# serycjon/MFT

Measured on AMD Instinct MI355X. Metric: tracked frames/sec at 512x512, 12 RAFT iters; flow EPE vs reference, higher is better.
Workload: dtype f32 (update-block products as split fp16 x 3 on the fp16 matrix cores, fp32 accumulation; error per product <= ~2^-23, see DESIGN.md section 4 and parity below); 1 GPU; MFT.track on synthetic 512x512 video, deltas [inf,1,2,4,8,16,32], 7/7.00/7 (min/mean/max) flow pairs per timed frame, 12 RAFT iters, seeded synthetic weights (BASELINE.json configs[1]); parallelism=single GPU, frames_resident_in_hbm=True, preroll_frames=32

## Files before the change

mft_amd/csrc/volume_tile.hip:

```cpp
#include "common.h"
#include "profile.h"
#include "device_prims.h"

namespace mftx {

constexpr int VT_C = 256;
constexpr int VT_ROW = VT_C * 4 + 16;
constexpr int VT_TARGETS = 128 * VT_ROW;
constexpr int VT_LDS = VT_TARGETS + 8 * 1024;

struct VolTileArgs {
    const float *f1;
    const float *f2s;
    float *lvl0, *lvl1, *lvl2, *lvl3;
    long long s0, s1, s2, s3;
    int P, N, h, w, sbw, n_sb, wb0;
    float scale;
    int qchunks, blocks_per_chunk;
    int ablate;
    int gathered;
    long long f2_bstride;
    PairPtrs f1p;
};

template <int N>
__device__ __forceinline__ float vt_shl(float v) {
    return __builtin_bit_cast(float, __builtin_amdgcn_update_dpp(0, __builtin_bit_cast(int, v), 0x100 + N, 0xf, 0xf, true));
}
template <int N>
__device__ __forceinline__ float vt_shr(float v) {
    return __builtin_bit_cast(float, __builtin_amdgcn_update_dpp(0, __builtin_bit_cast(int, v), 0x110 + N, 0xf, 0xf, true));
}

template <bool QSPLIT>
__global__ __launch_bounds__(512, 2) void volume_tile_kernel(VolTileArgs p) {
    extern __shared__ __attribute__((aligned(16))) unsigned char vt_lds[];
    unsigned char *lds = vt_lds;
    const int tid = (int)threadIdx.x, lane = tid & 63, wv = __builtin_amdgcn_readfirstlane(tid >> 6);
    const int wg = (int)blockIdx.x;
    const int qc = wg % p.qchunks, sb = (wg / p.qchunks) % p.n_sb, bz = wg / (p.qchunks * p.n_sb);
    const int sby = sb / p.sbw, sbx = sb - sby * p.sbw;
    const float k2048 = __builtin_bit_cast(float, __builtin_amdgcn_readfirstlane(0x45000000));

    {
        const float *f2p = p.f2s + (long long)bz * p.f2_bstride;
#pragma unroll 4
        for (int k = 0; k < 16; ++k) {
            const int q = k * 512 + tid, m = q >> 6, pc = q & 63;
            const int j = m >> 5, mm = m & 31;
            const int ty = 8 * sby + 4 * (j >> 1) + (mm >> 3), tx = 16 * sbx + 8 * (j & 1) + (mm & 7);
            uint4 v = make_uint4(0u, 0u, 0u, 0u);
            if (ty < p.h && tx < p.w) v = *reinterpret_cast<const uint4 *>(f2p + ((long long)ty * p.w + tx) * VT_C + pc * 4);
            *reinterpret_cast<uint4 *>(lds + m * VT_ROW + pc * 16) = v;
        }
    }
    lds_barrier();

    const unsigned char *abase = lds + (lane & 31) * VT_ROW + (lane >> 5) * 32;
    const int n_blocks = (p.N + 31) >> 5;
    const int b_lo = qc * p.blocks_per_chunk, b_hi = (b_lo + p.blocks_per_chunk < n_blocks) ? b_lo + p.blocks_per_chunk : n_blocks;
    const long long qbase = (long long)bz * p.N;
    const float inv2048 = 1.f / 2048.f;
    const int hf = lane >> 5;
    const int h2 = p.h >> 2, w2 = p.w >> 2, h3 = p.h >> 3, w3 = p.w >> 3;

    const int pp = lane & 31;
    const int l1_src = 4 * (32 * hf + 2 * (pp & 3) + 16 * ((pp >> 3) & 1) + ((pp >> 2) & 1) + 8 * (pp >> 4));
    const int l3_src = 4 * ((lane + 16) & 63);
    constexpr int PF = 3;
    f32x4 raw[PF][2];
    const float *f1base = p.gathered ? p.f1p.p[bz] : p.f1 + qbase * VT_C;
    auto row_of = [&](int qb) {
        const int q = qb * 32 + (lane & 31);
        return f1base + (long long)(q < p.N ? q : p.N - 1) * VT_C + 8 * hf;
    };
    auto prefetch = [&](const float *src) {
#pragma unroll
        for (int g = 0; g < PF; ++g) {
            raw[g][0] = *reinterpret_cast<const f32x4 *>(src + 16 * g);
            raw[g][1] = *reinterpret_cast<const f32x4 *>(src + 16 * g + 4);
        }
    };
    if (b_lo + wv < b_hi) prefetch(row_of(b_lo + wv));
    for (int qb = b_lo + wv; qb < b_hi; qb += 8) {
        const float *src = row_of(qb);
        f32x16 acc[4], accx[4];
#pragma unroll
        for (int j = 0; j < 4; ++j)
#pragma unroll
            for (int r = 0; r < 16; ++r) { acc[j][r] = 0.f; accx[j][r] = 0.f; }
        f16x8 ah[2][4], al[2][4];
        auto read_a = [&](int g, int set) {
#pragma unroll
            for (int j = 0; j < 4; ++j) {
                ah[set][j] = *reinterpret_cast<const f16x8 *>(abase + j * 32 * VT_ROW + g * 64);
                al[set][j] = *reinterpret_cast<const f16x8 *>(abase + j * 32 * VT_ROW + g * 64 + 16);
            }
        };
        read_a(0, 0);
#pragma unroll
        for (int g = 0; g < 16; ++g) {
            const int set = g & 1;
            f16x8 bh, bl;
            if constexpr (QSPLIT) {
                bh = __builtin_bit_cast(f16x8, raw[g % PF][0]);
                bl = __builtin_bit_cast(f16x8, raw[g % PF][1]);
            } else split8(raw[g % PF][0], raw[g % PF][1], k2048, bh, bl);
            __builtin_amdgcn_sched_barrier(0);
            if (g + 1 < 16) read_a(g + 1, set ^ 1);
            if (g + PF < 16) {
                raw[g % PF][0] = *reinterpret_cast<const f32x4 *>(src + 16 * (g + PF));
                raw[g % PF][1] = *reinterpret_cast<const f32x4 *>(src + 16 * (g + PF) + 4);
            }
            __builtin_amdgcn_sched_barrier(0);
#pragma unroll
            for (int j = 0; j < 4; ++j) acc[j] = mfma_f16(bh, ah[set][j], acc[j]);
#pragma unroll
            for (int j = 0; j < 4; ++j) accx[j] = mfma_f16(bh, al[set][j], accx[j]);
#pragma unroll
            for (int j = 0; j < 4; ++j) accx[j] = mfma_f16(bl, ah[set][j], accx[j]);
            __builtin_amdgcn_sched_barrier(0);
        }

        if (qb + 8 < b_hi) prefetch(row_of(qb + 8));
        __builtin_amdgcn_sched_barrier(0);

        const int m = lane & 31;
        const int q0 = qb * 32;
        const long long blk0 = ((long long)(2 * sby) * p.wb0 + 2 * sbx) * 32 + m;
        const int rows_ok = p.N - q0 < 32 ? p.N - q0 : 32;
        const __amdgpu_buffer_rsrc_t r0 = __builtin_amdgcn_make_buffer_rsrc(p.lvl0 + (qbase + q0) * p.s0, 0, (unsigned)((long long)rows_ok * p.s0 * 4), 0x00020000);
        const __amdgpu_buffer_rsrc_t r1 = __builtin_amdgcn_make_buffer_rsrc(p.lvl1 + (qbase + q0) * p.s1, 0, (unsigned)((long long)rows_ok * p.s1 * 4), 0x00020000);
        const unsigned v1off = (unsigned)((4 * hf * p.s1 + ((long long)sby * p.sbw + sbx) * 32 + m) * 4);
        const unsigned s0b = (unsigned)(p.s0 * 4), s1b = (unsigned)(p.s1 * 4), jrow = (unsigned)(p.wb0 * 128);
        int le = lane;
        asm volatile("" : "+v"(le));
        const int d2c = le & 7, d2hf = (le >> 3) & 1, d2i = le >> 4;
        const int l2_pull = 4 * (32 * d2hf + 16 * (d2c >> 2) + 2 * (d2c & 3));
        const int l2_y = 2 * sby + (d2c >> 2), l2_x = 4 * sbx + (d2c & 3);
        const bool l2_ok = l2_y < h2 && l2_x < w2;
        const int l2_off = l2_y * w2 + l2_x, l2_row = 4 * d2hf + d2i;
        const int d3c = le & 1, d3hf = (le >> 1) & 1, d3r = le >> 2;
        const int l3_pull = 4 * (32 * d3hf + 4 * d3c);
        const int l3_x = 2 * sbx + d3c;
        const bool l3_ok = sby < h3 && l3_x < w3;
        const int l3_off = sby * w3 + l3_x, l3_row = 8 * (d3r >> 2) + 4 * d3hf + (d3r & 3);
        float *slab = reinterpret_cast<float *>(lds + VT_TARGETS + wv * 1024);
        const unsigned v0off4 = (unsigned)((le >> 3) * s0b) + (unsigned)((blk0 - m) * 4) + (unsigned)(le & 7) * 16u;
        float acc2 = 0.f, acc3 = 0.f;
#pragma unroll
        for (int g = 0; g < 4; ++g) {
#ifdef MFTX_TUNING
            const bool st0g = !(p.ablate & 1);
#else
            const bool st0g = true;
#endif
            float vv[4][4];
#pragma unroll
            for (int i = 0; i < 4; ++i)
#pragma unroll
                for (int j = 0; j < 4; ++j) vv[i][j] = (acc[j][4 * g + i] + accx[j][4 * g + i] * inv2048) * p.scale;
            f32x4 line[4];
#pragma unroll
            for (int j = 0; j < 4; ++j) {
#pragma unroll
                for (int i = 0; i < 4; ++i) slab[(4 * hf + i) * 32 + m] = vv[i][j];
                line[j] = *reinterpret_cast<const f32x4 *>(slab + (le >> 3) * 32 + (le & 7) * 4);
            }
            if (st0g) {
#pragma unroll
                for (int j = 0; j < 4; ++j)
                    __builtin_amdgcn_raw_buffer_store_b128(__builtin_bit_cast(u32x4, line[j]), r0, v0off4 + (j >> 1) * jrow + (j & 1) * 128u, (unsigned)(8 * g) * s0b, 0);
            }
#pragma unroll
        for (int i = 0; i < 4; ++i) {
            const int r = 4 * g + i;
            const int qrow = q0 + 8 * (r >> 2) + 4 * hf + (r & 3);
            const bool row_ok = qrow < p.N;
#ifdef MFTX_TUNING
            const bool st1 = row_ok && !(p.ablate & 2);
#define MFTX_VT_ST23 (!(p.ablate & 10))
#else
            const bool st1 = row_ok;
#define MFTX_VT_ST23 true
#endif
            float merged = 0.f;
#pragma unroll
            for (int j = 0; j < 4; ++j) {
                const float v = vv[i][j];
                float t = v + vt_shl<1>(v);
                t = t + vt_shl<8>(v);
                t = (t + vt_shl<9>(v)) * 0.25f;
                if (j == 0) merged = t;
                else {
                    float sh = j == 1 ? vt_shr<1>(t) : (j == 2 ? vt_shr<8>(t) : vt_shr<9>(t));
                    asm volatile("" : "+v"(sh));
                    const bool take = j == 1 ? (m & 1) != 0 : (j == 2 ? ((m >> 3) & 1) && !(m & 1) : ((m >> 3) & 1) && (m & 1));
                    merged = take ? sh : merged;
                }
            }
            const float l1 = __builtin_bit_cast(float, __builtin_amdgcn_ds_bpermute(l1_src, __builtin_bit_cast(int, merged)));
            if (st1) __builtin_amdgcn_raw_buffer_store_b32(__builtin_bit_cast(unsigned, l1), r1, v1off, (unsigned)(8 * (r >> 2) + (r & 3)) * s1b, 0);
            float t2 = l1 + vt_shl<1>(l1);
            t2 = t2 + vt_shl<8>(l1);
            t2 = (t2 + vt_shl<9>(l1)) * 0.25f;
            asm volatile("" : "+v"(t2));
            {
                const float pulled = __builtin_bit_cast(float, __builtin_amdgcn_ds_bpermute(l2_pull, __builtin_bit_cast(int, t2)));
                acc2 = d2i == (r & 3) ? pulled : acc2;
                if ((r & 3) == 3) {
                    const int row2 = q0 + 8 * (r >> 2) + l2_row;
                    if (MFTX_VT_ST23 && l2_ok && row2 < p.N) p.lvl2[(qbase + row2) * p.s2 + l2_off] = acc2;
                }
            }
            const float bq = vt_shl<2>(t2);
            const float cq = __builtin_bit_cast(float, __builtin_amdgcn_ds_bpermute(l3_src, __builtin_bit_cast(int, t2)));
            const float dq = __builtin_bit_cast(float, __builtin_amdgcn_ds_bpermute(l3_src + 8, __builtin_bit_cast(int, t2)));
            float v3 = (((t2 + bq) + cq) + dq) * 0.25f;
            asm volatile("" : "+v"(v3));
            {
                const float pulled = __builtin_bit_cast(float, __builtin_amdgcn_ds_bpermute(l3_pull, __builtin_bit_cast(int, v3)));
                acc3 = d3r == r ? pulled : acc3;
                if (r == 15) {
                    const int row3 = q0 + l3_row;
                    if (MFTX_VT_ST23 && l3_ok && row3 < p.N) p.lvl3[(qbase + row3) * p.s3 + l3_off] = acc3;
                }
            }
        }
        }
    }
}

static int vt_num_cus() {
    static const int n = [] {
        int dev = 0, cus = 256;
        hipDeviceProp_t prop;
        if (hipGetDevice(&dev) == hipSuccess && hipGetDeviceProperties(&prop, dev) == hipSuccess && prop.multiProcessorCount > 0) cus = prop.multiProcessorCount;
        return cus;
    }();
    return n;
}

bool volume_tile_applicable(int C) { return C == VT_C; }

__global__ void vt_query_split_kernel(const float *__restrict__ in, uint4 *__restrict__ out, long long n8) {
    const long long i = (long long)blockIdx.x * blockDim.x + threadIdx.x;
    const float k2048 = __builtin_bit_cast(float, __builtin_amdgcn_readfirstlane(0x45000000));
    if (i >= n8) return;
    const f32x4 u = *reinterpret_cast<const f32x4 *>(in + i * 8), v = *reinterpret_cast<const f32x4 *>(in + i * 8 + 4);
    f16x8 hi, lo;
    split8(u, v, k2048, hi, lo);
    out[2 * i] = __builtin_bit_cast(uint4, hi);
    out[2 * i + 1] = __builtin_bit_cast(uint4, lo);
}

int launch_volume_query_split(const float *in, void *out, long long n, hipStream_t s) {
    if (n <= 0 || n % 8) return fail(MFTX_E_ARG, "volume_query_split: a positive multiple of 8 floats");
    if (!aligned16(in) || !aligned16(out)) return fail(MFTX_E_ALIGN, "volume_query_split: operands must be 16-byte aligned");
    const long long n8 = n / 8;
    hipLaunchKernelGGL(vt_query_split_kernel, dim3((unsigned)((n8 + 255) / 256)), dim3(256), 0, s, in, reinterpret_cast<uint4 *>(out), n8);
    return check_launch("volume_query_split");
}

int launch_volume_tile(const float *f1, const float *f2s, int P, int h, int w, float *const lvl[4], hipStream_t s, const PairPtrs *f1p, long long f2_bstride,
                       bool f1_split) {
    if (f1p && P > MFTX_MAX_GATHER) return fail(MFTX_E_ARG, "corr_pyramid: at most %d gathered pairs", MFTX_MAX_GATHER);
    const PyramidLayout L = pyramid_layout(h, w);
    VolTileArgs a{};
    a.f1 = f1; a.f2s = f2s; a.lvl0 = lvl[0]; a.lvl1 = lvl[1]; a.lvl2 = lvl[2]; a.lvl3 = lvl[3];
    a.s0 = L.stride[0]; a.s1 = L.stride[1]; a.s2 = L.stride[2]; a.s3 = L.stride[3];
    a.P = P; a.N = h * w; a.h = h; a.w = w; a.sbw = L.sbw; a.n_sb = L.sbh * L.sbw; a.wb0 = L.wb[0];
    a.scale = 1.0f / sqrtf((float)VT_C);
    a.gathered = f1p ? 1 : 0;
    if (f1p) a.f1p = *f1p;
    a.f2_bstride = f2_bstride >= 0 ? f2_bstride : (long long)a.N * VT_C;
    const int n_blocks = (a.N + 31) / 32;
    const long long base = (long long)P * a.n_sb;
    a.ablate = tune_env("MFTX_VT_ABLATE", 0);
    static const int q_forced = tune_env("MFTX_VT_QCHUNKS", 0);
    int qchunks = q_forced > 0 ? q_forced : (base * 4 >= 3LL * vt_num_cus() ? 1 : (int)((vt_num_cus() + base - 1) / base));
    if (qchunks < 1) qchunks = 1;
    if (qchunks > (n_blocks + 7) / 8) qchunks = (n_blocks + 7) / 8;
    a.blocks_per_chunk = (n_blocks + qchunks - 1) / qchunks;
    a.qchunks = (n_blocks + a.blocks_per_chunk - 1) / a.blocks_per_chunk;
    const long long wgs = base * a.qchunks;
    if (wgs > 0x7fffffffLL) return fail(MFTX_E_ARG, "corr_pyramid: too many workgroups");
    static bool attr_set = false;
    if (!attr_set) {
        if (hipFuncSetAttribute(reinterpret_cast<const void *>(volume_tile_kernel<false>), hipFuncAttributeMaxDynamicSharedMemorySize, VT_LDS) != hipSuccess ||
            hipFuncSetAttribute(reinterpret_cast<const void *>(volume_tile_kernel<true>), hipFuncAttributeMaxDynamicSharedMemorySize, VT_LDS) != hipSuccess)
            return fail(MFTX_E_STATE, "corr_pyramid: cannot reserve %d bytes of LDS", VT_LDS);
        attr_set = true;
    }
    ProfScope prof(PC_CORR_VOLUME, s, 2.0 * a.N * a.N * (double)VT_C * P);
    if (f1_split) hipLaunchKernelGGL(volume_tile_kernel<true>, dim3((unsigned)wgs), dim3(512), VT_LDS, s, a);
    else hipLaunchKernelGGL(volume_tile_kernel<false>, dim3((unsigned)wgs), dim3(512), VT_LDS, s, a);
    return check_launch("volume_tile");
}

}
```

Measured before the change: 187.4 frames/s.

## Deepen query prefetch ring, reorder MFMA/LDS reads, vectorize level-1 stores

Enlarges the per-wave prefetch ring of query feature loads from 3 to 8 k-groups. The ring now rolls over into the next query block instead of reloading it at the end of the loop. A-operand LDS reads drop from double buffering to single buffers for the high and low halves, interleaved between the MFMA groups, which reduces register pressure. Level-1 pyramid outputs are staged through an LDS slab and written as 128-bit buffer stores instead of scalar stores, and the lvl0/lvl1 stores now carry a cache policy flag (value 2). The aim is to hide global load latency, widen the stores and cut write cache pollution, at the cost of more VGPRs for the ring and a changed row-bounds check that relies on the buffer resource limit.

```diff
diff --git a/mft_amd/csrc/volume_tile.hip b/mft_amd/csrc/volume_tile.hip
--- a/mft_amd/csrc/volume_tile.hip
+++ b/mft_amd/csrc/volume_tile.hip
@@ -8,6 +8,7 @@
 constexpr int VT_ROW = VT_C * 4 + 16;
 constexpr int VT_TARGETS = 128 * VT_ROW;
 constexpr int VT_LDS = VT_TARGETS + 8 * 1024;
+constexpr int VT_STORE_POLICY = 2;
 
 struct VolTileArgs {
     const float *f1;
@@ -61,80 +62,77 @@
     const int b_lo = qc * p.blocks_per_chunk, b_hi = (b_lo + p.blocks_per_chunk < n_blocks) ? b_lo + p.blocks_per_chunk : n_blocks;
     const long long qbase = (long long)bz * p.N;
     const float inv2048 = 1.f / 2048.f;
-    const int hf = lane >> 5;
     const int h2 = p.h >> 2, w2 = p.w >> 2, h3 = p.h >> 3, w3 = p.w >> 3;
 
-    const int pp = lane & 31;
-    const int l1_src = 4 * (32 * hf + 2 * (pp & 3) + 16 * ((pp >> 3) & 1) + ((pp >> 2) & 1) + 8 * (pp >> 4));
-    const int l3_src = 4 * ((lane + 16) & 63);
-    constexpr int PF = 3;
+    constexpr int PF = 8;
+    static_assert(16 % PF == 0, "the ring must close over a query block's 16 k groups");
     f32x4 raw[PF][2];
-    const float *f1base = p.gathered ? p.f1p.p[bz] : p.f1 + qbase * VT_C;
+    const unsigned char *f1base = reinterpret_cast<const unsigned char *>(p.gathered ? p.f1p.p[bz] : p.f1 + qbase * VT_C);
+    auto lane_again = [] { return (int)__builtin_amdgcn_mbcnt_hi(~0u, __builtin_amdgcn_mbcnt_lo(~0u, 0u)); };
     auto row_of = [&](int qb) {
-        const int q = qb * 32 + (lane & 31);
-        return f1base + (long long)(q < p.N ? q : p.N - 1) * VT_C + 8 * hf;
+        const int ln = lane_again();
+        const int q = qb * 32 + (ln & 31);
+        return (unsigned)(q < p.N ? q : p.N - 1) * (unsigned)(VT_C * 4) + 32u * (unsigned)(ln >> 5);
     };
-    auto prefetch = [&](const float *src) {
-#pragma unroll
-        for (int g = 0; g < PF; ++g) {
-            raw[g][0] = *reinterpret_cast<const f32x4 *>(src + 16 * g);
-            raw[g][1] = *reinterpret_cast<const f32x4 *>(src + 16 * g + 4);
-        }
+    auto request = [&](int slot, unsigned src, int g) {
+        raw[slot][0] = *reinterpret_cast<const f32x4 *>(f1base + src + 64 * g);
+        raw[slot][1] = *reinterpret_cast<const f32x4 *>(f1base + src + 64 * g + 16);
     };
-    if (b_lo + wv < b_hi) prefetch(row_of(b_lo + wv));
-    for (int qb = b_lo + wv; qb < b_hi; qb += 8) {
-        const float *src = row_of(qb);
+    auto do_block = [&](const int qb) __attribute__((always_inline)) {
+        unsigned src = row_of(qb);
         f32x16 acc[4], accx[4];
 #pragma unroll
         for (int j = 0; j < 4; ++j)
 #pragma unroll
             for (int r = 0; r < 16; ++r) { acc[j][r] = 0.f; accx[j][r] = 0.f; }
-        f16x8 ah[2][4], al[2][4];
-        auto read_a = [&](int g, int set) {
-#pragma unroll
-            for (int j = 0; j < 4; ++j) {
-                ah[set][j] = *reinterpret_cast<const f16x8 *>(abase + j * 32 * VT_ROW + g * 64);
-                al[set][j] = *reinterpret_cast<const f16x8 *>(abase + j * 32 * VT_ROW + g * 64 + 16);
-            }
+        f16x8 ah[4], al[4];
+        auto read_al = [&](int g) {
+#pragma unroll
+            for (int j = 0; j < 4; ++j) al[j] = *reinterpret_cast<const f16x8 *>(abase + j * 32 * VT_ROW + g * 64 + 16);
         };
-        read_a(0, 0);
+        auto read_ah = [&](int g) {
+#pragma unroll
+            for (int j = 0; j < 4; ++j) ah[j] = *reinterpret_cast<const f16x8 *>(abase + j * 32 * VT_ROW + g * 64);
+        };
+        read_al(0);
+        read_ah(0);
 #pragma unroll
         for (int g = 0; g < 16; ++g) {
-            const int set = g & 1;
             f16x8 bh, bl;
             if constexpr (QSPLIT) {
                 bh = __builtin_bit_cast(f16x8, raw[g % PF][0]);
                 bl = __builtin_bit_cast(f16x8, raw[g % PF][1]);
             } else split8(raw[g % PF][0], raw[g % PF][1], k2048, bh, bl);
             __builtin_amdgcn_sched_barrier(0);
-            if (g + 1 < 16) read_a(g + 1, set ^ 1);
-            if (g + PF < 16) {
-                raw[g % PF][0] = *reinterpret_cast<const f32x4 *>(src + 16 * (g + PF));
-                raw[g % PF][1] = *reinterpret_cast<const f32x4 *>(src + 16 * (g + PF) + 4);
-            }
-            __builtin_amdgcn_sched_barrier(0);
-#pragma unroll
-            for (int j = 0; j < 4; ++j) acc[j] = mfma_f16(bh, ah[set][j], acc[j]);
-#pragma unroll
-            for (int j = 0; j < 4; ++j) accx[j] = mfma_f16(bh, al[set][j], accx[j]);
-#pragma unroll
-            for (int j = 0; j < 4; ++j) accx[j] = mfma_f16(bl, ah[set][j], accx[j]);
+            if (g == 16 - PF) src = qb + 8 < b_hi ? row_of(qb + 8) : 0u;
+            if constexpr (!QSPLIT) request(g % PF, src, (g + PF) % 16);
+            __builtin_amdgcn_sched_barrier(0);
+#pragma unroll
+            for (int j = 0; j < 4; ++j) accx[j] = mfma_f16(bh, al[j], accx[j]);
+            __builtin_amdgcn_sched_barrier(0);
+            if (g + 1 < 16) read_al(g + 1);
+            __builtin_amdgcn_sched_barrier(0);
+#pragma unroll
+            for (int j = 0; j < 4; ++j) acc[j] = mfma_f16(bh, ah[j], acc[j]);
+#pragma unroll
+            for (int j = 0; j < 4; ++j) accx[j] = mfma_f16(bl, ah[j], accx[j]);
+            __builtin_amdgcn_sched_barrier(0);
+            if (g + 1 < 16) read_ah(g + 1);
+            if constexpr (QSPLIT) request(g % PF, src, (g + PF) % 16);
             __builtin_amdgcn_sched_barrier(0);
         }
 
-        if (qb + 8 < b_hi) prefetch(row_of(qb + 8));
-        __builtin_amdgcn_sched_barrier(0);
-
-        const int m = lane & 31;
+        int le = lane_again();
+        asm volatile("" : "+v"(le));
+        const int m = le & 31, hf = le >> 5;
+        const int l1_src = 4 * (32 * hf + 2 * (m & 3) + 16 * ((m >> 3) & 1) + ((m >> 2) & 1) + 8 * (m >> 4));
+        const int l3_src = 4 * ((le + 16) & 63);
         const int q0 = qb * 32;
         const long long blk0 = ((long long)(2 * sby) * p.wb0 + 2 * sbx) * 32 + m;
         const int rows_ok = p.N - q0 < 32 ? p.N - q0 : 32;
         const __amdgpu_buffer_rsrc_t r0 = __builtin_amdgcn_make_buffer_rsrc(p.lvl0 + (qbase + q0) * p.s0, 0, (unsigned)((long long)rows_ok * p.s0 * 4), 0x00020000);
         const __amdgpu_buffer_rsrc_t r1 = __builtin_amdgcn_make_buffer_rsrc(p.lvl1 + (qbase + q0) * p.s1, 0, (unsigned)((long long)rows_ok * p.s1 * 4), 0x00020000);
-        const unsigned v1off = (unsigned)((4 * hf * p.s1 + ((long long)sby * p.sbw + sbx) * 32 + m) * 4);
         const unsigned s0b = (unsigned)(p.s0 * 4), s1b = (unsigned)(p.s1 * 4), jrow = (unsigned)(p.wb0 * 128);
-        int le = lane;
-        asm volatile("" : "+v"(le));
         const int d2c = le & 7, d2hf = (le >> 3) & 1, d2i = le >> 4;
         const int l2_pull = 4 * (32 * d2hf + 16 * (d2c >> 2) + 2 * (d2c & 3));
         const int l2_y = 2 * sby + (d2c >> 2), l2_x = 4 * sbx + (d2c & 3);
@@ -147,6 +145,7 @@
         const int l3_off = sby * w3 + l3_x, l3_row = 8 * (d3r >> 2) + 4 * d3hf + (d3r & 3);
         float *slab = reinterpret_cast<float *>(lds + VT_TARGETS + wv * 1024);
         const unsigned v0off4 = (unsigned)((le >> 3) * s0b) + (unsigned)((blk0 - m) * 4) + (unsigned)(le & 7) * 16u;
+        const unsigned v1off4 = (unsigned)((le >> 3) * s1b) + (unsigned)(((long long)sby * p.sbw + sbx) * 128) + (unsigned)(le & 7) * 16u;
         float acc2 = 0.f, acc3 = 0.f;
 #pragma unroll
         for (int g = 0; g < 4; ++g) {
@@ -170,18 +169,14 @@
             if (st0g) {
 #pragma unroll
                 for (int j = 0; j < 4; ++j)
-                    __builtin_amdgcn_raw_buffer_store_b128(__builtin_bit_cast(u32x4, line[j]), r0, v0off4 + (j >> 1) * jrow + (j & 1) * 128u, (unsigned)(8 * g) * s0b, 0);
+                    __builtin_amdgcn_raw_buffer_store_b128(__builtin_bit_cast(u32x4, line[j]), r0, v0off4 + (j >> 1) * jrow + (j & 1) * 128u, (unsigned)(8 * g) * s0b, VT_STORE_POLICY);
             }
 #pragma unroll
         for (int i = 0; i < 4; ++i) {
             const int r = 4 * g + i;
-            const int qrow = q0 + 8 * (r >> 2) + 4 * hf + (r & 3);
-            const bool row_ok = qrow < p.N;
 #ifdef MFTX_TUNING
-            const bool st1 = row_ok && !(p.ablate & 2);
 #define MFTX_VT_ST23 (!(p.ablate & 10))
 #else
-            const bool st1 = row_ok;
 #define MFTX_VT_ST23 true
 #endif
             float merged = 0.f;
@@ -200,7 +195,7 @@
                 }
             }
             const float l1 = __builtin_bit_cast(float, __builtin_amdgcn_ds_bpermute(l1_src, __builtin_bit_cast(int, merged)));
-            if (st1) __builtin_amdgcn_raw_buffer_store_b32(__builtin_bit_cast(unsigned, l1), r1, v1off, (unsigned)(8 * (r >> 2) + (r & 3)) * s1b, 0);
+            slab[(4 * hf + i) * 32 + m] = l1;
             float t2 = l1 + vt_shl<1>(l1);
             t2 = t2 + vt_shl<8>(l1);
             t2 = (t2 + vt_shl<9>(l1)) * 0.25f;
@@ -227,7 +222,24 @@
                 }
             }
         }
+            {
+                const f32x4 line1 = *reinterpret_cast<const f32x4 *>(slab + (le >> 3) * 32 + (le & 7) * 4);
+#ifdef MFTX_TUNING
+                const bool st1 = !(p.ablate & 2);
+#else
+                const bool st1 = true;
+#endif
+                if (st1) __builtin_amdgcn_raw_buffer_store_b128(__builtin_bit_cast(u32x4, line1), r1, v1off4, (unsigned)(8 * g) * s1b, VT_STORE_POLICY);
+            }
         }
+    };
+    const int qb0 = b_lo + wv;
+    if (qb0 < b_hi) {
+        const unsigned src0 = row_of(qb0);
+#pragma unroll
+        for (int g = 0; g < PF; ++g) request(g, src0, g);
+        do_block(qb0);
+        for (int qb = qb0 + 8; qb < b_hi; qb += 8) do_block(qb);
     }
 }
 
```

Result: no change. 187.9 frames/s, median of 6 (+0.3%).
